# Draghoyns/FLAIR-1

Measured on AMD Instinct MI355X. Metric: 512x512x5 tiles/s (train fwd+bwd), higher is better.
Workload: dtype bf16; 1 GPU; U-Net/ResNet34 5-ch 512x512 13-class train step (fwd + fused CE/argmax/confmat + bwd + SGD), bs=32/GPU, random-init weights; global_batch=32, parallelism=dp1, grad_allreduce=none

## Files before the change

flair-1_amd/csrc/conv_hg.hip:

```cpp
#include <stdlib.h>

#include "common.h"
#include "conv_route.h"
#include "halo_stage.h"
#include "launch.h"
#include "mma.h"
#include "tile_store.h"
#include "tune.h"

namespace flair {
namespace {

__device__ __forceinline__ int sw_off(int row, int chunk) { return row * 128 + ((chunk ^ (row & 7)) << 4); }

template <typename T, int TW, int TH, int BN, int HB, int TMv = 4>
struct HgCfg {
  static constexpr int CH = Elem<T>::CH;
  static constexpr int CK = 8 * CH;
  static constexpr int TPIX = TW * TH;
  static constexpr int HW_ = TW + 2, HH = TH + 2, HPIX = HW_ * HH;
  static constexpr int WMN = TPIX / (16 * TMv), WNN = BN / 64;
  static constexpr int NWAVE = WMN * WNN;
  static constexpr int NT = 64 * NWAVE;
  static constexpr int HALO = HPIX * 128;
// ... 169 lines not shown
#pragma unroll
  for (int q = 0; q < TN; ++q) {
    const int col = wn * 64 + q * 16 + lr;
    const bool cin_ok = (n0 + col) < a.Cout;
    const float osc = (a.oscale && cin_ok) ? a.oscale[n0 + col] : 1.f;
    const float bias = ((a.bias && cin_ok) ? a.bias[n0 + col] : 0.f) + ((a.oshift && cin_ok) ? a.oshift[n0 + col] : 0.f);
#pragma unroll
    for (int i = 0; i < TM; ++i) {
#pragma unroll
      for (int rr = 0; rr < 4; ++rr) {
        const int g = wm * TM + i;
        const int row = (g / MTX) * TW + (g % MTX) * 16 + lq * 4 + rr;
        T v = Elem<T>::from_f(fmaf(acc[i][q][rr], osc, bias));
        const float vf = Elem<T>::to_f(v);
        s1[q] += vf;
        s2[q] += vf * vf;
        *reinterpret_cast<T*>(ct + row * Cfg::CLD + col * (int)sizeof(T)) = v;
      }
    }
  }
  if (a.stats) {
#pragma unroll
    for (int q = 0; q < TN; ++q) {
      s1[q] += __shfl_xor(s1[q], 16); s1[q] += __shfl_xor(s1[q], 32);
      s2[q] += __shfl_xor(s2[q], 16); s2[q] += __shfl_xor(s2[q], 32);
      if (lq == 0) {
        st[(wm * BN + wn * 64 + q * 16 + lr) * 2 + 0] = s1[q];
        st[(wm * BN + wn * 64 + q * 16 + lr) * 2 + 1] = s2[q];
      }
    }
  }
  __syncthreads();
  if (a.stats) tile_stats_write<Cfg::WMN, BN>(st, a.stats, a.Cout, n0, ntiles, tile, t);
  store_tile<T, TW, TPIX, BN, NT, Cfg::CLD, BNR>(a, ct, n, y0, x0, n0, t, tile, ntiles);
}

void* g_debug_buffer = nullptr;
typedef const __attribute__((address_space(1))) void* gptr_t;
typedef __attribute__((address_space(3))) void* lptr_t;

template <typename T, int TW, int TH, int BN, int HB, int NS>
struct HgdCfg {
  static constexpr int CH = Elem<T>::CH;
  static constexpr int CK = 8 * CH;
  static constexpr int TPIX = TW * TH;
  static constexpr int HW_ = TW + 2, HH = TH + 2, HPIX = HW_ * HH;
  static constexpr int WMN = TPIX / 64, WNN = BN >= 64 ? BN / 64 : 1;
  static constexpr int TN = BN / 16 / WNN;
  static constexpr int NWAVE = WMN * WNN;
  static constexpr int NT = 64 * NWAVE;
  static constexpr int HALO = HPIX * 128;
  static constexpr int BTILE = BN * 128;
  static constexpr int CLD = BN * (int)sizeof(T) + 16;
  static constexpr int CT = TPIX * CLD;
  static constexpr int STAGES = HB * HALO + NS * BTILE;
  static constexpr int MAIN = STAGES > CT ? STAGES : CT;
  static constexpr int STATS = WMN * BN * 2 * 4;
  static constexpr int SMEM = MAIN + STATS;
  static constexpr int HITEMS = (HPIX * 8 + NT - 1) / NT;
  static constexpr int DPW = BTILE / (1024 * NWAVE);
  static constexpr int D = NS - 1;
  static_assert(BTILE % (1024 * NWAVE) == 0, "every wave streams whole 1 KiB pieces");
  static_assert(D >= 1 && D <= 3, "ring depth");
};

__device__ __forceinline__ void wait_vm_lgkm0(int n) {
#define FLAIR_VM_CASE(k) case k: asm volatile("s_waitcnt vmcnt(" #k ") lgkmcnt(0)" ::: "memory"); break;
  switch (n) {
    FLAIR_VM_CASE(1) FLAIR_VM_CASE(2) FLAIR_VM_CASE(3) FLAIR_VM_CASE(4) FLAIR_VM_CASE(5) FLAIR_VM_CASE(6) FLAIR_VM_CASE(7)
    FLAIR_VM_CASE(8) FLAIR_VM_CASE(9) FLAIR_VM_CASE(10) FLAIR_VM_CASE(11) FLAIR_VM_CASE(12) FLAIR_VM_CASE(13)
    FLAIR_VM_CASE(14) FLAIR_VM_CASE(15) FLAIR_VM_CASE(16) FLAIR_VM_CASE(17) FLAIR_VM_CASE(18) FLAIR_VM_CASE(19)
    FLAIR_VM_CASE(20) FLAIR_VM_CASE(21) FLAIR_VM_CASE(22) FLAIR_VM_CASE(23) FLAIR_VM_CASE(24) FLAIR_VM_CASE(25)
    FLAIR_VM_CASE(26) FLAIR_VM_CASE(27) FLAIR_VM_CASE(28) FLAIR_VM_CASE(29) FLAIR_VM_CASE(30) FLAIR_VM_CASE(31)
    FLAIR_VM_CASE(32) FLAIR_VM_CASE(33) FLAIR_VM_CASE(34) FLAIR_VM_CASE(35) FLAIR_VM_CASE(36) FLAIR_VM_CASE(37)
    FLAIR_VM_CASE(38) FLAIR_VM_CASE(39) FLAIR_VM_CASE(40) FLAIR_VM_CASE(41) FLAIR_VM_CASE(42) FLAIR_VM_CASE(43)
    FLAIR_VM_CASE(44) FLAIR_VM_CASE(45) FLAIR_VM_CASE(46) FLAIR_VM_CASE(47) FLAIR_VM_CASE(48)
    default: asm volatile("s_waitcnt vmcnt(0) lgkmcnt(0)" ::: "memory"); break;
  }
#undef FLAIR_VM_CASE
}

enum { XF_NONE = 0, XF_LAZY = 1 };

template <typename T, int TW, int TH, int BN, int HB, int NS, bool BNR, int XF>
__global__ __launch_bounds__(TW * TH * (BN >= 64 ? BN : 64) / 64, 2) void conv3x3_hgd_kernel(const ConvArgs a) {
  constexpr bool LAZY = XF == XF_LAZY;
  using Cfg = HgdCfg<T, TW, TH, BN, HB, NS>;
  constexpr int CH = Cfg::CH, CK = Cfg::CK, HW_ = Cfg::HW_, HPIX = Cfg::HPIX, NT = Cfg::NT, TPIX = Cfg::TPIX;
  constexpr int TM = 4, TN = Cfg::TN, MTX = TW / 16, DPW = Cfg::DPW, D = Cfg::D, HITEMS = Cfg::HITEMS;
  extern __shared__ __attribute__((aligned(16))) unsigned char smem[];
  unsigned char* halo0 = smem;
  unsigned char* bt0 = smem + HB * Cfg::HALO;
  const int t = threadIdx.x, lane = t & 63;
  const int wave = __builtin_amdgcn_readfirstlane(t >> 6);
  const int lr = lane & 15, lq = lane >> 4;
  const int wm = wave % Cfg::WMN, wn = wave / Cfg::WMN;
  const int H = a.Hout, W = a.Wout;
  const int tiles_x = W / TW, tiles_y = H / TH;
  const int NB = a.Cout / BN;
  const int nwork = gridDim.x;
  int w = blockIdx.x;
  if (a.xcd_remap) {
    const int q = nwork >> 3, r = nwork & 7, xcd = w & 7;
    w = (xcd < r ? xcd * (q + 1) : r * (q + 1) + (xcd - r) * q) + (w >> 3);
  }
  const int tile = w / NB;
  const int ntiles = nwork / NB;
  int n, y0, x0;
  tile_decode<TW, TH>(tile, tiles_x, tiles_y, n, y0, x0);
  const int n0 = (w - tile * NB) * BN;
  const int Cin = a.C0 + a.C1;
  const T* __restrict__ src0 = (const T*)a.src0;
  const T* __restrict__ src1 = (const T*)a.src1;
  const unsigned char* __restrict__ wp = (const unsigned char*)a.w;
  const int Hs0 = a.up0 ? (H >> 1) : H, Ws0 = a.up0 ? (W >> 1) : W;
  const int nchunks = Cin / CK;

  u32x4 hreg[HITEMS];
  unsigned hbits = 0;
  float lsc[CH], lsh[CH];
  bool hlazy = false;
  auto halo_load = [&](int chunk) {
    const int cbase = chunk * CK;
    const bool use0 = cbase < a.C0;
    const T* __restrict__ base = use0 ? src0 : src1;
    const int Hs = use0 ? Hs0 : H, Ws = use0 ? Ws0 : W, Cs = use0 ? a.C0 : a.C1;
    const int sh = (use0 && a.up0) ? 1 : 0;
    const int coff = use0 ? cbase : cbase - a.C0;
    unsigned hb2 = 0;
#pragma unroll
    for (int k = 0; k < HITEMS; ++k) {
      const int it = t + NT * k;
      const int hp = it >> 3, ch = it & 7;
      const int hy = hp / HW_, hx = hp - hy * HW_;
      const int iy = y0 - 1 + hy, ix = x0 - 1 + hx;
      const bool ok = (it < HPIX * 8) && ((unsigned)iy < (unsigned)H) && ((unsigned)ix < (unsigned)W);
      const unsigned off = ok ? (unsigned)(((n * Hs + (iy >> sh)) * Ws + (ix >> sh)) * Cs + coff + ch * CH) : 0u;
      hreg[k] = *reinterpret_cast<const u32x4*>(base + off);
      hb2 |= (ok ? 1u : 0u) << k;
    }
    hbits = hb2;
    if constexpr (LAZY) {
      hlazy = use0 && a.in_scale != nullptr;
      const int c0 = hlazy ? coff + (t & 7) * CH : 0;
      const float* __restrict__ ps = hlazy ? a.in_scale : (const float*)a.w;
      const float* __restrict__ ph = hlazy ? a.in_shift : (const float*)a.w;
#pragma unroll
      for (int e = 0; e < CH; e += 4) {
        const float4 v1 = *reinterpret_cast<const float4*>(ps + c0 + e), v2 = *reinterpret_cast<const float4*>(ph + c0 + e);
        lsc[e] = v1.x; lsc[e + 1] = v1.y; lsc[e + 2] = v1.z; lsc[e + 3] = v1.w;
        lsh[e] = v2.x; lsh[e + 1] = v2.y; lsh[e + 2] = v2.z; lsh[e + 3] = v2.w;
      }
    }
  };
  constexpr int HLOADS = HITEMS + (LAZY ? 2 * (CH / 4) : 0);
  static_assert((D - 1) * DPW + HLOADS <= 48, "wait_vm_lgkm0 covers the largest count its two call sites (prologue, end of a "
                                              "tap step) request: the D - 1 younger weight tiles and the loads of one halo chunk");
  auto halo_store = [&](int buf) {
    unsigned char* hb = halo0 + buf * Cfg::HALO;
#pragma unroll
    for (int k = 0; k < HITEMS; ++k) {
      const int it = t + NT * k;
      if (it < HPIX * 8) {
        const int hp = it >> 3, hx = hp % HW_;
        u32x4 v = hreg[k];
        if constexpr (LAZY) {
          if (hlazy) v = chunk_bn_relu<T, u32x4>(v, lsc, lsh);
        }
        *reinterpret_cast<u32x4*>(hb + hp * 128 + (((it & 7) ^ (hx & 7)) << 4)) = v & (0u - ((hbits >> k) & 1u));
        if constexpr (LAZY) __builtin_amdgcn_sched_barrier(0);
      }
    }
  };
  const unsigned bvo = (unsigned)(((n0 + wave * (DPW * 8) + (lane >> 3)) * a.Kpad + (((lane & 7) ^ (lane >> 3)) * CH)) * (int)sizeof(T));
  const unsigned brow = (unsigned)(8 * a.Kpad * (int)sizeof(T));
  auto b_dma = [&](int chunk, int tap, int slot) {
    const unsigned char* gb = wp + (size_t)(unsigned)((tap * Cin + chunk * CK) * (int)sizeof(T));
    unsigned char* lb = bt0 + slot * Cfg::BTILE + wave * (DPW * 1024);
#pragma unroll
    for (int j = 0; j < DPW; ++j)
      __builtin_amdgcn_global_load_lds((gptr_t)(gb + (bvo + j * brow)), (lptr_t)(lb + j * 1024), 16, 0, 0);
  };

  f32x4_t acc[TM][TN];
#pragma unroll
  for (int i = 0; i < TM; ++i)
#pragma unroll
    for (int j = 0; j < TN; ++j) acc[i][j] = f32x4_t{0.f, 0.f, 0.f, 0.f};

  unsigned abase[3], bfo[TN];
#pragma unroll
  for (int sx = 0; sx < 3; ++sx) abase[sx] = (unsigned)((lr + sx) * 128 + ((lq ^ ((lr + sx) & 7)) << 4));
#pragma unroll
  for (int j = 0; j < TN; ++j) bfo[j] = (unsigned)sw_off(wn * 64 + j * 16 + lr, lq);
  static_assert(TM % MTX == 0, "a wave's M tiles start at a tile-row boundary");
  const unsigned wbase = (unsigned)((wm * TM / MTX) * HW_ * 128);

  const int nsteps = 9 * nchunks;
  auto stamp = [&](int i) {
#ifdef FLAIR_HG_STAMPS
    if (a.dbg && t == 0) a.dbg[(size_t)blockIdx.x * 8 + i] = i == 5 || i == 6 ? __builtin_amdgcn_s_memrealtime() : __builtin_amdgcn_s_memtime();
#else
    (void)i;
#endif
  };
  stamp(0);
  stamp(5);
  u32x4 afA[TM], bfA[TN], afB[TM], bfB[TN];
  auto rd = [&](u32x4 (&af)[TM], u32x4 (&bf)[TN], const unsigned char* hbuf, int slot, int tap, int h) {
    const unsigned char* bb = bt0 + slot * Cfg::BTILE;
    const unsigned char* hbr = hbuf + (tap / 3) * (HW_ * 128);
#pragma unroll
    for (int j = 0; j < TN; ++j) bf[j] = *reinterpret_cast<const u32x4*>(bb + (bfo[j] ^ (h << 6)));
#pragma unroll
    for (int i = 0; i < TM; ++i)
      af[i] = *reinterpret_cast<const u32x4*>(hbr + wbase + ((i / MTX) * HW_ + (i % MTX) * 16) * 128 + (abase[tap % 3] ^ (h << 6)));
  };
  auto mm = [&](const u32x4 (&af)[TM], const u32x4 (&bf)[TN]) {
#pragma unroll
    for (int i = 0; i < TM; ++i)
#pragma unroll
      for (int j = 0; j < TN; ++j) Mma<T>::run(bf[j], af[i], acc[i][j]);
  };
  halo_load(0);
#pragma unroll
  for (int d = 0; d < D; ++d)
    if (d < nsteps) b_dma(d / 9, d % 9, d % NS);
  halo_store(0);
  const bool pre1 = nchunks > 1;
  if (pre1) halo_load(1);
  wait_vm_lgkm0((D - 1) * DPW + (pre1 ? HLOADS : 0));
  __builtin_amdgcn_s_barrier();
  __builtin_amdgcn_sched_barrier(0);
  stamp(1);
  constexpr bool PIPE = sizeof(T) == 2 && !(LAZY && BN == 64);
  if constexpr (PIPE) rd(afA, bfA, halo0, 0, 0, 0);

  int sb = 0;
  for (int chunk = 0; chunk < nchunks; ++chunk) {
    const unsigned char* hb = halo0 + (HB == 2 ? (chunk & 1) : 0) * Cfg::HALO;
    const unsigned char* hbn = halo0 + (HB == 2 ? ((chunk + 1) & 1) : 0) * Cfg::HALO;
    const bool last = chunk == nchunks - 1;
#pragma unroll
    for (int tap = 0; tap < 9; ++tap) {
      const int cur = (9 % NS == 0) ? (tap % NS) : ((sb + tap) % NS);
      const int nxt = (9 % NS == 0) ? ((tap + 1) % NS) : ((sb + tap + 1) % NS);
      {
        const int tp = tap + D;
        const int pc = tp >= 9 ? chunk + 1 : chunk, pt = tp >= 9 ? tp - 9 : tp;
        const int pslot = (9 % NS == 0) ? (tp % NS) : ((sb + tp) % NS);
        if (pc < nchunks) b_dma(pc, pt, pslot);
      }
      if constexpr (PIPE) {
        rd(afB, bfB, hb, cur, tap, 1);
        mm(afA, bfA);
      } else {
        rd(afA, bfA, hb, cur, tap, 0);
        mm(afA, bfA);
        rd(afA, bfA, hb, cur, tap, 1);
        mm(afA, bfA);
      }
      bool halo_younger = false;
      if (tap == 8) {
        if constexpr (HB == 2) {
          if (!last) {
            halo_store((chunk + 1) & 1);
            if (chunk + 2 < nchunks) { halo_load(chunk + 2); halo_younger = true; }
          }
        }
      } else if (tap <= D - 2) {
        halo_younger = chunk + 1 < nchunks;
      }
      const int left = last ? 8 - tap : 9;
      const int groups = left < 1 ? 0 : ((left < D ? left : D) - 1);
      wait_vm_lgkm0(left < 1 ? 0 : groups * DPW + (halo_younger ? HLOADS : 0));
      __builtin_amdgcn_s_barrier();
      __builtin_amdgcn_sched_barrier(0);
      if (tap < 8) {
        if constexpr (PIPE) {
          rd(afA, bfA, hb, nxt, tap + 1, 0);
          mm(afB, bfB);
        }
      } else if (!last) {
        if constexpr (HB == 1) {
          halo_store(0);
          if (chunk + 2 < nchunks) halo_load(chunk + 2);
          if constexpr (PIPE) mm(afB, bfB);
          asm volatile("s_waitcnt lgkmcnt(0)" ::: "memory");
          __builtin_amdgcn_s_barrier();
          __builtin_amdgcn_sched_barrier(0);
          if constexpr (PIPE) rd(afA, bfA, hbn, nxt, 0, 0);
        } else if constexpr (PIPE) {
          rd(afA, bfA, hbn, nxt, 0, 0);
          mm(afB, bfB);
        }
      } else if constexpr (PIPE) {
        mm(afB, bfB);
      }
    }
    if (9 % NS != 0) sb = (sb + 9) % NS;
  }
  stamp(2);

  unsigned char* ct = smem;
  float* st = reinterpret_cast<float*>(smem + Cfg::MAIN);
  const bool want_stats = a.stats != nullptr;
  const bool affine = a.oscale != nullptr || a.bias != nullptr || a.oshift != nullptr;
#pragma unroll
  for (int q = 0; q < TN; ++q) {
    const int colb = wn * 64 + q * 16 + lq * 4;
    float osc[4], bia[4];
#pragma unroll
    for (int rr = 0; rr < 4; ++rr) { osc[rr] = 1.f; bia[rr] = 0.f; }
    if (affine) {
#pragma unroll
      for (int rr = 0; rr < 4; ++rr) {
        const int c = n0 + colb + rr;
        const bool ok = c < a.Cout;
        if (a.oscale && ok) osc[rr] = a.oscale[c];
        bia[rr] = ((a.bias && ok) ? a.bias[c] : 0.f) + ((a.oshift && ok) ? a.oshift[c] : 0.f);
      }
    }
#pragma unroll
    for (int i = 0; i < TM; ++i) {
      const int g = wm * TM + i;
      const int row = (g / MTX) * TW + (g % MTX) * 16 + lr;
      float v[4];
#pragma unroll
      for (int rr = 0; rr < 4; ++rr) v[rr] = affine ? fmaf(acc[i][q][rr], osc[rr], bia[rr]) : acc[i][q][rr];
      if constexpr (sizeof(T) == 2) {
        uint2 pk;
        pk.x = (unsigned)f32_to_bf16(v[0]) | ((unsigned)f32_to_bf16(v[1]) << 16);
        pk.y = (unsigned)f32_to_bf16(v[2]) | ((unsigned)f32_to_bf16(v[3]) << 16);
        *reinterpret_cast<uint2*>(ct + row * Cfg::CLD + colb * 2) = pk;
      } else {
        *reinterpret_cast<float4*>(ct + row * Cfg::CLD + colb * 4) = make_float4(v[0], v[1], v[2], v[3]);
      }
    }
  }
  stamp(7);
  if (want_stats) {
    const unsigned char* cw = ct + (wm * 64) * Cfg::CLD + (wn * 64) * (int)sizeof(T);
#pragma unroll
    for (int q = 0; q < TN; ++q) {
      f32x4_t m1 = f32x4_t{0.f, 0.f, 0.f, 0.f}, m2 = f32x4_t{0.f, 0.f, 0.f, 0.f};
      if constexpr (sizeof(T) == 2) {
        typedef __attribute__((address_space(3))) s16x4_t* lds_p;
        const int p4 = lr & 3, q4 = lr >> 2;
#pragma unroll
        for (int ks = 0; ks < 2; ++ks) {
          const unsigned char* lo = cw + (ks * 32 + 8 * lq + q4) * Cfg::CLD + q * 32 + 8 * p4;
          const s16x4_t x0 = __builtin_amdgcn_ds_read_tr16_b64_v4i16((lds_p)(lo));
          const s16x4_t x1 = __builtin_amdgcn_ds_read_tr16_b64_v4i16((lds_p)(lo + 4 * Cfg::CLD));
          u32x4 xf;
          xf.x = (unsigned)(unsigned short)x0[0] | ((unsigned)(unsigned short)x0[1] << 16);
          xf.y = (unsigned)(unsigned short)x0[2] | ((unsigned)(unsigned short)x0[3] << 16);
          xf.z = (unsigned)(unsigned short)x1[0] | ((unsigned)(unsigned short)x1[1] << 16);
          xf.w = (unsigned)(unsigned short)x1[2] | ((unsigned)(unsigned short)x1[3] << 16);
          const u32x4 ones = u32x4{0x3F803F80u, 0x3F803F80u, 0x3F803F80u, 0x3F803F80u};
          Mma<T>::run(ones, xf, m1);
          Mma<T>::run(xf, xf, m2);
        }
      } else {
#pragma unroll
        for (int kk = 0; kk < 16; kk += 4) {
          u32x4 xf;
          xf.x = *reinterpret_cast<const unsigned*>(cw + ((kk + 0) * 4 + lq) * Cfg::CLD + (q * 16 + lr) * 4);
          xf.y = *reinterpret_cast<const unsigned*>(cw + ((kk + 1) * 4 + lq) * Cfg::CLD + (q * 16 + lr) * 4);
          xf.z = *reinterpret_cast<const unsigned*>(cw + ((kk + 2) * 4 + lq) * Cfg::CLD + (q * 16 + lr) * 4);
          xf.w = *reinterpret_cast<const unsigned*>(cw + ((kk + 3) * 4 + lq) * Cfg::CLD + (q * 16 + lr) * 4);
          const u32x4 ones = u32x4{0x3F800000u, 0x3F800000u, 0x3F800000u, 0x3F800000u};
          Mma<T>::run(ones, xf, m1);
          Mma<T>::run(xf, xf, m2);
        }
      }
      const int dr = lr & 3;
      const float d2 = dr == 0 ? m2[0] : dr == 1 ? m2[1] : dr == 2 ? m2[2] : m2[3];
      if (lq == 0) st[(wm * BN + wn * 64 + q * 16 + lr) * 2 + 0] = m1[0];
      if (lq == (lr >> 2)) st[(wm * BN + wn * 64 + q * 16 + lr) * 2 + 1] = d2;
    }
  }
  __syncthreads();
  if (a.stats) tile_stats_write<Cfg::WMN, BN>(st, a.stats, a.Cout, n0, ntiles, tile, t);
  stamp(3);
  store_tile<T, TW, TPIX, BN, NT, Cfg::CLD, BNR>(a, ct, n, y0, x0, n0, t, tile, ntiles);
  stamp(4);
  stamp(6);
}

static const char* hg_prof_name(size_t es, int BN) {
  static const char* names[2][3] = {{"conv3x3_hg_f32_n32", "conv3x3_hg_f32_n64", "conv3x3_hg_f32_n128"},
                                    {"conv3x3_hg_bf16_n32", "conv3x3_hg_bf16_n64", "conv3x3_hg_bf16_n128"}};
  return names[es == 2][BN == 128 ? 2 : BN == 64 ? 1 : 0];
}

template <typename T, int TW, int TH, int BN, int HB, int NS, bool BNR, int XF>
int launch_hgd_cfg_b(const ConvArgs& a, hipStream_t s) {
  using Cfg = HgdCfg<T, TW, TH, BN, HB, NS>;
  const long M = (long)a.N * a.Hout * a.Wout;
  dim3 grid((unsigned)(M / Cfg::TPIX) * (a.Cout / BN));
  ConvArgs b = a;
  b.xcd_remap = tune("FLAIR_XCD_REMAP", 1);
  b.dbg = (unsigned long long*)g_debug_buffer;
  return launch_kernel<conv3x3_hgd_kernel<T, TW, TH, BN, HB, NS, BNR, XF>>(hg_prof_name(sizeof(T), BN), conv_prof_cost(a, sizeof(T), true, false), grid,
                                                                           dim3(Cfg::NT), Cfg::SMEM, s, b);
}

template <typename T, int TW, int TH, int BN, int HB, int NS>
int launch_hgd_cfg(const ConvArgs& a, hipStream_t s) {
  if constexpr (BN == 32) {
    return (a.in_scale || a.bnr_partial) ? -6 : launch_hgd_cfg_b<T, TW, TH, BN, HB, NS, false, XF_NONE>(a, s);
  } else {
    if (a.in_scale) return a.bnr_partial ? -6 : launch_hgd_cfg_b<T, TW, TH, BN, HB, NS, false, XF_LAZY>(a, s);
    if constexpr (sizeof(T) == 2)
      return a.bnr_partial ? launch_hgd_cfg_b<T, TW, TH, BN, HB, NS, true, XF_NONE>(a, s)
                           : launch_hgd_cfg_b<T, TW, TH, BN, HB, NS, false, XF_NONE>(a, s);
    else
      return -6;
  }
}

int g_hg_variant = -1;

template <typename T, int TW, int TH, int BN, int HB, bool BNR, int TMv = 4>
int launch_hg_cfg_b(const ConvArgs& a, hipStream_t s) {
  using Cfg = HgCfg<T, TW, TH, BN, HB, TMv>;
  const long M = (long)a.N * a.Hout * a.Wout;
  dim3 grid((unsigned)(M / Cfg::TPIX) * (a.Cout / BN));
  ConvArgs b = a;
  b.xcd_remap = tune("FLAIR_XCD_REMAP", 1);
  return launch_kernel<conv3x3_hg_kernel<T, TW, TH, BN, HB, BNR, TMv>>(hg_prof_name(sizeof(T), BN), conv_prof_cost(a, sizeof(T), true, false), grid,
                                                                       dim3(Cfg::NT), Cfg::SMEM, s, b);
}

template <typename T, int TW, int TH, int BN, int HB, int TMv = 4>
int launch_hg_cfg(const ConvArgs& a, hipStream_t s) {
  return a.bnr_partial ? launch_hg_cfg_b<T, TW, TH, BN, HB, true, TMv>(a, s) : launch_hg_cfg_b<T, TW, TH, BN, HB, false, TMv>(a, s);
}

}

static int hg_dma_mode() { return tune("FLAIR_HG_DMA", 1); }

static int hg_tile_pixels(int dtype, const ConvArgs& a) {
  (void)dtype;
  if (g_hg_variant < 0) g_hg_variant = tune("FLAIR_HG_VARIANT", 1);
  const bool can128 = (a.Wout % 16 == 0) && (a.Hout % 8 == 0);
  const bool can256 = (a.Wout % 32 == 0 && a.Hout % 8 == 0) || (a.Wout % 16 == 0 && a.Hout % 16 == 0);
  if ((a.Cout % 128) != 0) return can256 ? 256 : (can128 ? 128 : 0);
  if (hg_dma_mode() == 0 && g_hg_variant == 0 && can256) return 256;
  if (can128) return 128;
  return can256 ? 256 : 0;
}

bool conv_hg_applicable(int dtype, const ConvArgs& a) {
  const int ck = dtype == DT_F32 ? 32 : 64;
  const int Cin = a.C0 + a.C1;
  if (a.R != 3 || a.S != 3 || a.out_mul != 1 || a.in_div != 1 || a.pad != 1) return false;
  if (a.Hout != a.Hin || a.Wout != a.Win || a.out_nchw || !a.out) return false;
  if (a.in_scale && (hg_dma_mode() == 0 || a.bnr_partial)) return false;
  if ((Cin % ck) || (a.C0 % ck)) return false;
  if (a.Cout == 32) return hg_dma_mode() != 0 && tune("FLAIR_HG_N32", 1) != 0 && !a.bnr_partial && !a.in_scale && a.pool_c0 == 0 &&
                           ((a.Wout % 32 == 0 && a.Hout % 8 == 0) || (a.Wout % 16 == 0 && a.Hout % 16 == 0));
  if (a.Cout < 64 || (a.Cout % 64)) return false;
  return hg_tile_pixels(dtype, a) != 0;
}

int conv_hg_grid_rows(int dtype, const ConvArgs& a) { return (int)((long)a.N * a.Hout * a.Wout / hg_tile_pixels(dtype, a)); }

template <typename T>
static int launch_hg_t(int tp, const ConvArgs& a, hipStream_t s) {
  const bool n128 = (a.Cout % 128) == 0;
  const int dma = hg_dma_mode();
  if (a.Cout == 32) {
    if (a.Wout % 32 == 0) return launch_hgd_cfg<T, 32, 8, 32, 1, 3>(a, s);
    return launch_hgd_cfg<T, 16, 16, 32, 1, 3>(a, s);
  }
  if (dma != 0 && (sizeof(T) == 2 || a.in_scale)) {
    if (tp == 128) return n128 ? launch_hgd_cfg<T, 16, 8, 128, 1, 3>(a, s) : launch_hgd_cfg<T, 16, 8, 64, 1, 3>(a, s);
    if (a.Wout % 32 == 0) return n128 ? launch_hgd_cfg<T, 32, 8, 128, 1, 3>(a, s) : launch_hgd_cfg<T, 32, 8, 64, 1, 3>(a, s);
    return n128 ? launch_hgd_cfg<T, 16, 16, 128, 1, 3>(a, s) : launch_hgd_cfg<T, 16, 16, 64, 1, 3>(a, s);
  }
  if (tp == 128) return n128 ? launch_hg_cfg<T, 16, 8, 128, 2>(a, s) : launch_hg_cfg<T, 16, 8, 64, 2>(a, s);
  if (a.Wout % 32 == 0) return n128 ? launch_hg_cfg<T, 32, 8, 128, 2>(a, s) : launch_hg_cfg<T, 32, 8, 64, 1>(a, s);
  return n128 ? launch_hg_cfg<T, 16, 16, 128, 2>(a, s) : launch_hg_cfg<T, 16, 16, 64, 1>(a, s);
}

int set_debug_buffer(void* p) {
#ifdef FLAIR_HG_STAMPS
  g_debug_buffer = p;
  return 0;
#else
  (void)p;
  return -7;
#endif
}

int launch_conv_hg(int dtype, const ConvArgs& a, hipStream_t s) {
  const int tp = hg_tile_pixels(dtype, a);
  return dtype == DT_F32 ? launch_hg_t<float>(tp, a, s) : launch_hg_t<bf16_t>(tp, a, s);
}

}
```

flair-1_amd/csrc/conv_igemm.hip:

```cpp
#include "common.h"
#include "conv_route.h"
#include "launch.h"
#include "mma.h"
#include "tile_store.h"
#include "tune.h"

namespace flair {

__device__ __forceinline__ int lds_off(int row, int chunk) { return row * 128 + ((chunk ^ (row & 7)) << 4); }

template <typename T, int BM, int BN, int WAVES_M, int WAVES_N>
struct ConvCfg {
  static constexpr int CH = Elem<T>::CH;
  static constexpr int BKE = 8 * CH;
  static constexpr int STAGE = (BM + BN) * 128;
  static constexpr int CLD = BN * (int)sizeof(T) + 16;
  static constexpr int CT = BM * CLD;
  static constexpr int MAIN = (2 * STAGE > CT) ? 2 * STAGE : CT;
  static constexpr int STATS = WAVES_M * BN * 2 * 4;
  static constexpr int SMEM = MAIN + STATS;
};

template <typename T, int BM, int BN, int WAVES_M, int WAVES_N>
__global__ __launch_bounds__(256, 2) void conv_igemm_kernel(const ConvArgs a) {
// ... 188 lines not shown
        uint4 v = *reinterpret_cast<const uint4*>(ct + row * Cfg::CLD + ch * 16);
        long mo = m;
        if (a.out_sub) {
          const int HWo = a.Hout * a.Wout;
          const int img = (int)(m / HWo), rem = (int)(m - (long)img * HWo);
          const int ho = rem / a.Wout, wo = rem - ho * a.Wout;
          mo = ((long)img * 2 * a.Hout + 2 * ho + c_oy) * (2 * a.Wout) + 2 * wo + c_ox;
        }
        T* dst = out + mo * a.out_ld + n;
        if (a.ores || a.orelu || a.ogelu) {
          float fa[CH];
          chunk_to_f<T>(v, fa);
          if (a.ogelu) {
#pragma unroll
            for (int e = 0; e < CH; ++e) fa[e] = 0.5f * fa[e] * (1.f + erff(fa[e] * 0.70710678118654752f));
          }
          if (a.ores) {
            float fb[CH];
            chunk_to_f<T>(*reinterpret_cast<const uint4*>((const T*)a.ores + mo * a.out_ld + n), fb);
#pragma unroll
            for (int e = 0; e < CH; ++e) fa[e] += fb[e];
          }
          if (a.orelu) {
#pragma unroll
            for (int e = 0; e < CH; ++e) fa[e] = fmaxf(fa[e], 0.f);
          }
          v = f_to_chunk<T>(fa);
        }
        if (a.accumulate) {
          uint4 o = *reinterpret_cast<const uint4*>(dst);
          float fa[CH], fb[CH];
          chunk_to_f<T>(v, fa);
          chunk_to_f<T>(o, fb);
#pragma unroll
          for (int e = 0; e < CH; ++e) fa[e] += fb[e];
          v = f_to_chunk<T>(fa);
        }
        *reinterpret_cast<uint4*>(dst) = v;
      }
    }
  }
  if (a.out_nchw) {
    const int HW = a.Hout * a.Wout;
    for (int idx = t; idx < BM * BN; idx += 256) {
      const int nl = idx / BM, ml = idx - nl * BM;
      const long m = m0 + ml;
      const int n = n0 + nl;
      if (m < M && n < a.Cout) {
        const long img = m / HW, pix = m - img * HW;
        a.out_nchw[(img * a.Cout + n) * HW + pix] =
            Elem<T>::to_f(*reinterpret_cast<const T*>(ct + ml * Cfg::CLD + nl * (int)sizeof(T)));
      }
    }
  }
}

template <typename T, int BM, int BN, int WAVES_M, int WAVES_N>
static int launch_cfg(const ConvArgs& a, hipStream_t s) {
  using Cfg = ConvCfg<T, BM, BN, WAVES_M, WAVES_N>;
  const long M = (long)a.N * a.Hout * a.Wout;
  dim3 grid(cdiv(M, BM), cdiv(a.Cout, BN), a.ncls ? a.ncls : 1);
  const double flops = 2.0 * (double)M * a.Cout * a.Kg / (a.in_div * a.in_div);
  const double bytes = ((double)a.N * a.Hin * a.Win / (a.in_div * a.in_div) / (a.up0 ? 4 : 1) * a.C0 +
                        (double)a.N * a.Hin * a.Win * a.C1 + (double)M * a.Cout * (a.accumulate ? 2 : 1)) * sizeof(T) +
                       (double)a.Cout * a.Kg * sizeof(T);
  static const char* names[2][4] = {{"conv_igemm_f32_128x128", "conv_igemm_f32_128x64", "conv_igemm_f32_256x32", "conv_igemm_f32_256x16"},
                                    {"conv_igemm_bf16_128x128", "conv_igemm_bf16_128x64", "conv_igemm_bf16_256x32", "conv_igemm_bf16_256x16"}};
  const int ci = BN == 128 ? 0 : BN == 64 ? 1 : BN == 32 ? 2 : 3;
  return launch_kernel<conv_igemm_kernel<T, BM, BN, WAVES_M, WAVES_N>>(names[sizeof(T) == 2][ci], ProfCost{flops, bytes}, grid, dim3(256), Cfg::SMEM, s, a);
}

static inline int pick_bn(int cout) { return cout >= 128 ? 128 : cout >= 64 ? 64 : cout >= 32 ? 32 : 16; }
static inline int pick_bm(int cout) { return cout >= 64 ? 128 : 256; }

ConvFamily conv_family(int dtype, const ConvArgs& a) {
  if (conv_stem_applicable(dtype, a)) return CONV_STEM;
  if (conv_hg_applicable(dtype, a)) return CONV_HG;
  if (conv_halo_applicable(a)) return CONV_HALO;
  return CONV_GATHER;
}

static bool tile_epilogue_ok(ConvFamily f, const ConvArgs& a) {
  if ((a.Hout & 1) || (a.Wout & 1)) return false;
  if (f == CONV_HG) return a.pool_c0 % ((a.Cout % 128) == 0 ? 128 : 64) == 0;
  if (f == CONV_HALO) return a.pool_c0 % (a.Cout <= 16 ? 16 : 32) == 0 && !a.out_nchw;
  return false;
}

bool conv_tile_epilogue_ok(int dtype, const ConvArgs& a) { return tile_epilogue_ok(conv_family(dtype, a), a); }

bool conv_mfma_bound(int dtype, const ConvArgs& a) {
  const int mode = tune("FLAIR_BNR", 2);
  if (mode == 0) return false;
  if (conv_family(dtype, a) != CONV_HG) return conv_halo_bnr_applicable(a);
  return mode == 2 || (a.Cout % 128) == 0;
}

bool conv_acc_src_ok(int dtype, const ConvArgs& a) { return a.acc_src && a.accumulate && a.pool_c0 == 0 && conv_family(dtype, a) == CONV_HG; }

int conv_grid_rows(int dtype, const ConvArgs& a) {
  switch (conv_family(dtype, a)) {
    case CONV_STEM: return conv_stem_grid_rows(a);
    case CONV_HG: return conv_hg_grid_rows(dtype, a);
    case CONV_HALO: return conv_halo_grid_rows(dtype, a);
    default: return cdiv((long)a.N * a.Hout * a.Wout, pick_bm(a.Cout));
  }
}

int conv_weight_rows_pad(int cout) { return (int)round_up(cout, pick_bn(cout)); }

template <typename T>
static int launch_t(const ConvArgs& a, hipStream_t s) {
  constexpr int CH = Elem<T>::CH;
  if ((a.C0 % CH) || (a.C1 % CH) || (a.Kpad % (8 * CH))) return -2;
  if (a.ncls && (a.ncls != 4 || !a.out_sub)) return -2;
  for (int c = 0; c < a.ncls; ++c)
    if (!a.cls_w[c] || (a.cls_kpad[c] % (8 * CH))) return -2;
  if (a.out && (a.Cout % CH)) return -3;
  if (a.up0 && ((a.Hin | a.Win) & 1)) return -4;
  if (a.in_div != 1 && a.in_div != 2) return -5;
  const long M = (long)a.N * a.Hout * a.Wout;
  const int bn = pick_bn(a.Cout);
  const bool small = !a.stats && !a.ncls && bn >= 64 && a.Kpad >= 8 * 8 * Elem<T>::CH && (long)cdiv(M, 128) * cdiv(a.Cout, bn) < 256 &&
                     tune("FLAIR_IGEMM_BM32", 2);
  if (small) {
    const int mode = tune("FLAIR_IGEMM_BM32", 2);
    if (mode >= 2 && (long)cdiv(M, 32) * cdiv(a.Cout, bn) < 512) return launch_cfg<T, 32, 32, 2, 2>(a, s);
    return bn == 128 ? launch_cfg<T, 32, 128, 2, 2>(a, s) : launch_cfg<T, 32, 64, 2, 2>(a, s);
  }
  switch (bn) {
    case 128: return launch_cfg<T, 128, 128, 2, 2>(a, s);
    case 64: return launch_cfg<T, 128, 64, 4, 1>(a, s);
    case 32: return launch_cfg<T, 256, 32, 4, 1>(a, s);
    default: return launch_cfg<T, 256, 16, 4, 1>(a, s);
  }
}

int launch_conv(int dtype, const ConvArgs& a, hipStream_t s) {
  const ConvFamily f = conv_family(dtype, a);
  if (a.preds_u8 && !conv_halo_preds_ok(dtype, a)) return -6;
  if (a.ce_lab8 && !conv_halo_ce_ok(dtype, a)) return -6;
  if (a.out_sub && (a.out_nchw || a.stats || a.pool_c0 > 0 || a.bnr_partial || f != CONV_GATHER)) return -6;
  if ((a.acc_src || a.bnr_mask) && f != CONV_HG) return -6;
  if (a.acc_src && !(a.accumulate && a.pool_c0 == 0)) return -6;
  if (a.bnr_mask && !a.bnr_partial) return -6;
  if (a.ogelu && (!a.out || a.out_nchw || a.in_scale || f != CONV_GATHER)) return -6;
  if (a.in_scale && ((f != CONV_HG && f != CONV_HALO) || (f == CONV_HG && (a.pool_c0 > 0 || a.bnr_partial)))) return -6;
  const bool tile_ok = tile_epilogue_ok(f, a);
  if (a.pool_c0 > 0 && !tile_ok) return -6;
  if (a.bnr_partial && !a.in_scale && !(tile_ok && (f == CONV_HG || conv_halo_bnr_applicable(a)))) return -6;
  switch (f) {
    case CONV_STEM: return launch_conv_stem(a, s);
    case CONV_HG: return launch_conv_hg(dtype, a, s);
    case CONV_HALO: {
      const int ch = dtype == DT_F32 ? 4 : 8;
      if (a.out && (a.Cout % ch) && a.out_ld < (int)round_up(a.Cout, ch)) return -3;
      return launch_conv_halo(dtype, a, s);
    }
    default: return dtype == DT_F32 ? launch_t<float>(a, s) : launch_t<bf16_t>(a, s);
  }
}

}
```

flair-1_amd/csrc/tile_store.h:

```cpp
#pragma once
#include "common.h"

namespace flair {

template <typename T, int TPIX, int BN, int NT>
struct TileItems {
  static constexpr int CH = Elem<T>::CH, CPR = BN / CH, ITEMS = (TPIX * CPR + NT - 1) / NT;
};

template <typename T, int TW, int TPIX, int BN, int NT>
__device__ __forceinline__ void tile_bnr_prefetch(const ConvArgs& a, int n, int y0, int x0, int n0, int t,
                                                  uint4 (&yv)[TileItems<T, TPIX, BN, NT>::ITEMS],
                                                  uint4 (&ov)[TileItems<T, TPIX, BN, NT>::ITEMS]) {
  using TI = TileItems<T, TPIX, BN, NT>;
  constexpr int CH = TI::CH, CPR = TI::CPR;
  const int H = a.Hout, W = a.Wout;
#pragma unroll
  for (int k = 0; k < TI::ITEMS; ++k) {
    const int idx = t + k * NT;
    const int row = idx / CPR, ch = idx - row * CPR;
    const int py = row / TW, px = row - py * TW;
    const int nn = n0 + ch * CH;
    const bool ok = idx < TPIX * CPR && nn < a.Cout;
    const long goff = ok ? ((long)(n * H + y0 + py) * W + x0 + px) * a.out_ld + nn : 0;
// ... 84 lines not shown
          float fb[CH];
          chunk_to_f<T>(*reinterpret_cast<const uint4*>(ct + row * CLD + ch * 16), fb);
#pragma unroll
          for (int e = 0; e < CH; ++e) fa[e] += fb[e];
        }
        T* dst = out + ((long)(n * Hh + (y0 >> 1) + py2) * Wh + (x0 >> 1) + px2) * a.out_ld + nn;
        if (a.accumulate) {
          float fb[CH];
          chunk_to_f<T>(*reinterpret_cast<const uint4*>(dst), fb);
#pragma unroll
          for (int e = 0; e < CH; ++e) fa[e] += fb[e];
        }
        uint4 v = f_to_chunk<T>(fa);
        if (bnr) v = bnr_item(v, *reinterpret_cast<const uint4*>((const T*)a.bnr_y + (dst - out)),
                              a.bnr_out ? *reinterpret_cast<const uint4*>((const T*)a.bnr_out + (dst - out)) : v);
        *reinterpret_cast<uint4*>(dst) = v;
      }
    }
    if (bnr) bnr_finish();
    return;
  }
  T* __restrict__ out = (T*)(a.pool_c0 > 0 ? a.out_skip : a.out);
  if (!out) return;
  const int ld = a.pool_c0 > 0 ? a.out_skip_ld : a.out_ld;
  const int cbase = a.pool_c0 > 0 ? a.pool_c0 : 0;
  const int acc = a.pool_c0 > 0 ? a.skip_accumulate : a.accumulate;
  constexpr int ITEMS = TileItems<T, TPIX, BN, NT>::ITEMS;
  uint4 yv[ITEMS], ov[ITEMS], av[ITEMS];
  if (bnr) tile_bnr_prefetch<T, TW, TPIX, BN, NT>(a, n, y0, x0, n0, t, yv, ov);
  const T* asrc = (a.acc_src && a.pool_c0 == 0) ? (const T*)a.acc_src : out;
  if (acc) {
#pragma unroll
    for (int k = 0; k < ITEMS; ++k) {
      const int idx = t + k * NT;
      const int row = idx / CPR, ch = idx - row * CPR;
      const int py = row / TW, px = row - py * TW;
      const int nn = n0 + ch * CH;
      const bool ok = idx < TPIX * CPR && nn < a.Cout;
      const long goff = ok ? ((long)(n * H + y0 + py) * W + x0 + px) * ld + (nn - cbase) : 0;
      av[k] = *reinterpret_cast<const uint4*>(asrc + goff);
    }
  }
#pragma unroll
  for (int k = 0; k < ITEMS; ++k) {
    const int idx = t + k * NT;
    if (idx >= TPIX * CPR) break;
    const int row = idx / CPR, ch = idx - row * CPR;
    const int py = row / TW, px = row - py * TW;
    const int nn = n0 + ch * CH;
    if (nn < a.Cout) {
      uint4 v = *reinterpret_cast<const uint4*>(ct + row * CLD + ch * 16);
      const long goff = ((long)(n * H + y0 + py) * W + x0 + px) * ld + (nn - cbase);
      T* dst = out + goff;
      if (a.ores || a.orelu) {
        float fa[CH];
        chunk_to_f<T>(v, fa);
        if (a.ores) {
          float fb[CH];
          chunk_to_f<T>(*reinterpret_cast<const uint4*>((const T*)a.ores + goff), fb);
#pragma unroll
          for (int e = 0; e < CH; ++e) fa[e] += fb[e];
        }
        if (a.orelu) {
#pragma unroll
          for (int e = 0; e < CH; ++e) fa[e] = fmaxf(fa[e], 0.f);
        }
        v = f_to_chunk<T>(fa);
      }
      if (acc) {
        float fa[CH], fb[CH];
        chunk_to_f<T>(v, fa);
        chunk_to_f<T>(av[k], fb);
#pragma unroll
        for (int e = 0; e < CH; ++e) fa[e] += fb[e];
        v = f_to_chunk<T>(fa);
      }
      if (bnr) v = bnr_item(v, yv[k], ov[k]);
      *reinterpret_cast<uint4*>(dst) = v;
    }
  }
  if (bnr) bnr_finish();
}

}
```

Measured before the change: 2835 tiles/s.

## Route stride-2 3x3 convs and their sub-pixel dgrad through the halo MFMA kernel

Adds stride-2 variants of the halo-DMA conv kernel. Forward stride-2 3x3 convs load the input as four polyphase sub-grids with a reordered tap table, so each halo chunk is reused across the taps of its phase. The backward data-gradient is split into four output-parity classes, each a small dense conv written by a new sub-pixel tile store. Both paths previously went through slower generic kernels; the new code adds more kernel instantiations and extra barriers at halo swaps.

```diff
diff --git a/flair-1_amd/csrc/conv_hg.hip b/flair-1_amd/csrc/conv_hg.hip
--- a/flair-1_amd/csrc/conv_hg.hip
+++ b/flair-1_amd/csrc/conv_hg.hip
@@ -275,9 +275,35 @@
 
 enum { XF_NONE = 0, XF_LAZY = 1 };
 
-template <typename T, int TW, int TH, int BN, int HB, int NS, bool BNR, int XF>
+enum { S2_NONE = 0, S2_FWD = 1, S2_DGRAD = 2 };
+constexpr int s2_period(int mode) { return mode == 0 ? 9 : mode == 1 ? 1 : mode == 4 ? 4 : 2; }
+constexpr int s2_groups(int mode) { return mode == 0 ? 4 : 1; }
+constexpr int s2_wtap(int mode, int k) {
+  constexpr int fwd[9] = {0, 2, 6, 8, 3, 5, 1, 7, 4};
+  return mode == 0 ? fwd[k] : k;
+}
+constexpr int s2_halo_tap(int mode, int k) {
+  if (mode == 0) return (s2_wtap(0, k) / 3 ? 3 : 0) + (s2_wtap(0, k) % 3 ? 1 : 0);
+  const int cs = ((mode - 1) & 1) ? 2 : 1;
+  return (1 + k / cs) * 3 + 1 + k % cs;
+}
+constexpr bool s2_group_end(int mode, int k) { return mode == 0 ? (k == 3 || k == 5 || k == 7 || k == 8) : k == s2_period(mode) - 1; }
+
+constexpr unsigned long long s2_pack(int mode, bool halo) {
+  unsigned long long v = 0;
+  for (int k = 0; k < s2_period(mode); ++k) v |= (unsigned long long)(halo ? s2_halo_tap(mode, k) : s2_wtap(mode, k)) << (4 * k);
+  return v;
+}
+constexpr unsigned s2_gmask(int mode) {
+  unsigned v = 0;
+  for (int k = 0; k < s2_period(mode); ++k) v |= (s2_group_end(mode, k) ? 1u : 0u) << k;
+  return v;
+}
+
+template <typename T, int TW, int TH, int BN, int HB, int NS, bool BNR, int XF, int S2 = S2_NONE>
 __global__ __launch_bounds__(TW * TH * (BN >= 64 ? BN : 64) / 64, 2) void conv3x3_hgd_kernel(const ConvArgs a) {
   constexpr bool LAZY = XF == XF_LAZY;
+  static_assert(S2 == S2_NONE || (HB == 1 && NS == 3 && !BNR && sizeof(T) == 2), "stride-2 flavours: single halo buffer, bf16");
   using Cfg = HgdCfg<T, TW, TH, BN, HB, NS>;
   constexpr int CH = Cfg::CH, CK = Cfg::CK, HW_ = Cfg::HW_, HPIX = Cfg::HPIX, NT = Cfg::NT, TPIX = Cfg::TPIX;
   constexpr int TM = 4, TN = Cfg::TN, MTX = TW / 16, DPW = Cfg::DPW, D = Cfg::D, HITEMS = Cfg::HITEMS;
@@ -305,7 +331,9 @@
   const int Cin = a.C0 + a.C1;
   const T* __restrict__ src0 = (const T*)a.src0;
   const T* __restrict__ src1 = (const T*)a.src1;
-  const unsigned char* __restrict__ wp = (const unsigned char*)a.w;
+  const int cls = S2 == S2_DGRAD ? 3 - (int)blockIdx.z : 0;
+  const unsigned char* __restrict__ wp = (const unsigned char*)(S2 == S2_DGRAD ? a.cls_w[cls] : a.w);
+  const int kpad = S2 == S2_DGRAD ? a.cls_kpad[cls] : a.Kpad;
   const int Hs0 = a.up0 ? (H >> 1) : H, Ws0 = a.up0 ? (W >> 1) : W;
   const int nchunks = Cin / CK;
 
@@ -313,9 +341,11 @@
   unsigned hbits = 0;
   float lsc[CH], lsh[CH];
   bool hlazy = false;
-  auto halo_load = [&](int chunk) {
-    const int cbase = chunk * CK;
-    const bool use0 = cbase < a.C0;
+  auto halo_load = [&](int chunk) __attribute__((always_inline)) {
+    const int pl = S2 == S2_FWD ? (chunk & 3) : 0;
+    const int pr = (pl & 1) ^ 1, pc = pl < 2 ? 1 : 0;
+    const int cbase = (S2 == S2_FWD ? (chunk >> 2) : chunk) * CK;
+    const bool use0 = S2 != S2_NONE || cbase < a.C0;
     const T* __restrict__ base = use0 ? src0 : src1;
     const int Hs = use0 ? Hs0 : H, Ws = use0 ? Ws0 : W, Cs = use0 ? a.C0 : a.C1;
     const int sh = (use0 && a.up0) ? 1 : 0;
@@ -327,8 +357,15 @@
       const int hp = it >> 3, ch = it & 7;
       const int hy = hp / HW_, hx = hp - hy * HW_;
       const int iy = y0 - 1 + hy, ix = x0 - 1 + hx;
-      const bool ok = (it < HPIX * 8) && ((unsigned)iy < (unsigned)H) && ((unsigned)ix < (unsigned)W);
-      const unsigned off = ok ? (unsigned)(((n * Hs + (iy >> sh)) * Ws + (ix >> sh)) * Cs + coff + ch * CH) : 0u;
+      bool ok = (it < HPIX * 8) && ((unsigned)iy < (unsigned)H) && ((unsigned)ix < (unsigned)W);
+      unsigned off;
+      if constexpr (S2 == S2_FWD) {
+        ok = ok && hy <= TH && hx <= TW && (hy >= 1 || pr) && (hx >= 1 || pc);
+        off = ok ? (unsigned)(((n * 2 * H + 2 * iy + pr) * (2 * W) + 2 * ix + pc) * Cs + coff + ch * CH) : 0u;
+      } else {
+        if constexpr (S2 == S2_DGRAD) ok = ok && hy >= 1 && hx >= 1;
+        off = ok ? (unsigned)(((n * Hs + (iy >> sh)) * Ws + (ix >> sh)) * Cs + coff + ch * CH) : 0u;
+      }
       hreg[k] = *reinterpret_cast<const u32x4*>(base + off);
       hb2 |= (ok ? 1u : 0u) << k;
     }
@@ -349,7 +386,7 @@
   constexpr int HLOADS = HITEMS + (LAZY ? 2 * (CH / 4) : 0);
   static_assert((D - 1) * DPW + HLOADS <= 48, "wait_vm_lgkm0 covers the largest count its two call sites (prologue, end of a "
                                               "tap step) request: the D - 1 younger weight tiles and the loads of one halo chunk");
-  auto halo_store = [&](int buf) {
+  auto halo_store = [&](int buf) __attribute__((always_inline)) {
     unsigned char* hb = halo0 + buf * Cfg::HALO;
 #pragma unroll
     for (int k = 0; k < HITEMS; ++k) {
@@ -365,9 +402,9 @@
       }
     }
   };
-  const unsigned bvo = (unsigned)(((n0 + wave * (DPW * 8) + (lane >> 3)) * a.Kpad + (((lane & 7) ^ (lane >> 3)) * CH)) * (int)sizeof(T));
-  const unsigned brow = (unsigned)(8 * a.Kpad * (int)sizeof(T));
-  auto b_dma = [&](int chunk, int tap, int slot) {
+  const unsigned bvo = (unsigned)(((n0 + wave * (DPW * 8) + (lane >> 3)) * kpad + (((lane & 7) ^ (lane >> 3)) * CH)) * (int)sizeof(T));
+  const unsigned brow = (unsigned)(8 * kpad * (int)sizeof(T));
+  auto b_dma = [&](int chunk, int tap, int slot) __attribute__((always_inline)) {
     const unsigned char* gb = wp + (size_t)(unsigned)((tap * Cin + chunk * CK) * (int)sizeof(T));
     unsigned char* lb = bt0 + slot * Cfg::BTILE + wave * (DPW * 1024);
 #pragma unroll
@@ -400,7 +437,7 @@
   stamp(0);
   stamp(5);
   u32x4 afA[TM], bfA[TN], afB[TM], bfB[TN];
-  auto rd = [&](u32x4 (&af)[TM], u32x4 (&bf)[TN], const unsigned char* hbuf, int slot, int tap, int h) {
+  auto rd = [&](u32x4 (&af)[TM], u32x4 (&bf)[TN], const unsigned char* hbuf, int slot, int tap, int h) __attribute__((always_inline)) {
     const unsigned char* bb = bt0 + slot * Cfg::BTILE;
     const unsigned char* hbr = hbuf + (tap / 3) * (HW_ * 128);
 #pragma unroll
@@ -409,12 +446,88 @@
     for (int i = 0; i < TM; ++i)
       af[i] = *reinterpret_cast<const u32x4*>(hbr + wbase + ((i / MTX) * HW_ + (i % MTX) * 16) * 128 + (abase[tap % 3] ^ (h << 6)));
   };
-  auto mm = [&](const u32x4 (&af)[TM], const u32x4 (&bf)[TN]) {
+  auto mm = [&](const u32x4 (&af)[TM], const u32x4 (&bf)[TN]) __attribute__((always_inline)) {
 #pragma unroll
     for (int i = 0; i < TM; ++i)
 #pragma unroll
       for (int j = 0; j < TN; ++j) Mma<T>::run(bf[j], af[i], acc[i][j]);
   };
+  constexpr bool PIPE = sizeof(T) == 2 && !(LAZY && BN == 64) && !(S2 == S2_FWD && BN == 64);
+  if constexpr (S2 != S2_NONE) {
+  static_assert(D == 2, "the look-ahead below is written for the ring of three");
+  unsigned long long wtab = s2_pack(0, false), htab = s2_pack(0, true);
+  unsigned gmask = s2_gmask(0);
+  int P = s2_period(0);
+  if constexpr (S2 == S2_DGRAD) {
+    P = cls == 0 ? s2_period(1) : cls == 3 ? s2_period(4) : s2_period(2);
+    wtab = s2_pack(4, false);
+    htab = cls == 0 ? s2_pack(1, true) : cls == 1 ? s2_pack(2, true) : cls == 2 ? s2_pack(3, true) : s2_pack(4, true);
+    gmask = 1u << (P - 1);
+  }
+  auto wtap_of = [&](int k) __attribute__((always_inline)) { return (int)((wtab >> (4 * k)) & 15); };
+  auto htap_of = [&](int k) __attribute__((always_inline)) { return (int)((htab >> (4 * k)) & 15); };
+  auto rdr = [&](u32x4 (&af)[TM], u32x4 (&bf)[TN], int slot, int htap, int h) __attribute__((always_inline)) {
+    const int hr = htap >= 6 ? 2 : htap >= 3 ? 1 : 0, hs = htap - 3 * hr;
+    const unsigned asel = (hs == 0 ? abase[0] : hs == 1 ? abase[1] : abase[2]) ^ (unsigned)(h << 6);
+    const unsigned char* bb = bt0 + slot * Cfg::BTILE;
+    const unsigned char* hbr = halo0 + hr * (HW_ * 128) + wbase;
+#pragma unroll
+    for (int j = 0; j < TN; ++j) bf[j] = *reinterpret_cast<const u32x4*>(bb + (bfo[j] ^ (h << 6)));
+#pragma unroll
+    for (int i = 0; i < TM; ++i) af[i] = *reinterpret_cast<const u32x4*>(hbr + ((i / MTX) * HW_ + (i % MTX) * 16) * 128 + asel);
+  };
+  const int nst = P * nchunks, nhalo = (S2 == S2_FWD ? s2_groups(0) : 1) * nchunks;
+  halo_load(0);
+  b_dma(0, wtap_of(0), 0);
+  if (nst > 1) b_dma(P == 1 ? 1 : 0, wtap_of(P == 1 ? 0 : 1), 1);
+  halo_store(0);
+  bool hyoung = nhalo > 1;
+  if (hyoung) halo_load(1);
+  wait_vm_lgkm0((nst > 1 ? DPW : 0) + (hyoung ? HLOADS : 0));
+  __builtin_amdgcn_s_barrier();
+  __builtin_amdgcn_sched_barrier(0);
+  if constexpr (PIPE) rdr(afA, bfA, 0, htap_of(0), 0);
+  int q = 0, k = 0, slot = 0, hidx = 0;
+#pragma unroll 1
+  for (int left = nst - 1; left >= 0; --left) {
+    int k1 = k + 1, q1 = q;
+    if (k1 == P) { k1 = 0; ++q1; }
+    int k2 = k1 + 1, q2 = q1;
+    if (k2 == P) { k2 = 0; ++q2; }
+    const int nxt = slot + 1 == NS ? 0 : slot + 1, pslot = nxt + 1 == NS ? 0 : nxt + 1;
+    if (q2 < nchunks) b_dma(q2, wtap_of(k2), pslot);
+    const int htap = htap_of(k);
+    if constexpr (PIPE) {
+      rdr(afB, bfB, slot, htap, 1);
+      mm(afA, bfA);
+    } else {
+      rdr(afA, bfA, slot, htap, 0);
+      mm(afA, bfA);
+      rdr(afA, bfA, slot, htap, 1);
+      mm(afA, bfA);
+    }
+    wait_vm_lgkm0(left < 1 ? 0 : (left >= D ? DPW : 0) + (hyoung ? HLOADS : 0));
+    hyoung = false;
+    __builtin_amdgcn_s_barrier();
+    __builtin_amdgcn_sched_barrier(0);
+    const bool sw = ((gmask >> k) & 1u) != 0 && left >= 1;
+    if (sw) {
+      halo_store(0);
+      ++hidx;
+      if (hidx + 1 < nhalo) { halo_load(hidx + 1); hyoung = true; }
+    } else if (left >= 1) {
+      if constexpr (PIPE) rdr(afA, bfA, nxt, htap_of(k1), 0);
+    }
+    if constexpr (PIPE) mm(afB, bfB);
+    if (sw) {
+      asm volatile("s_waitcnt lgkmcnt(0)" ::: "memory");
+      __builtin_amdgcn_s_barrier();
+      __builtin_amdgcn_sched_barrier(0);
+      if constexpr (PIPE) rdr(afA, bfA, nxt, htap_of(k1), 0);
+    }
+    k = k1; q = q1; slot = nxt;
+  }
+  } else {
   halo_load(0);
 #pragma unroll
   for (int d = 0; d < D; ++d)
@@ -426,7 +539,6 @@
   __builtin_amdgcn_s_barrier();
   __builtin_amdgcn_sched_barrier(0);
   stamp(1);
-  constexpr bool PIPE = sizeof(T) == 2 && !(LAZY && BN == 64);
   if constexpr (PIPE) rd(afA, bfA, halo0, 0, 0, 0);
 
   int sb = 0;
@@ -493,6 +605,7 @@
     }
     if (9 % NS != 0) sb = (sb + 9) % NS;
   }
+  }
   stamp(2);
 
   unsigned char* ct = smem;
@@ -576,7 +689,8 @@
   __syncthreads();
   if (a.stats) tile_stats_write<Cfg::WMN, BN>(st, a.stats, a.Cout, n0, ntiles, tile, t);
   stamp(3);
-  store_tile<T, TW, TPIX, BN, NT, Cfg::CLD, BNR>(a, ct, n, y0, x0, n0, t, tile, ntiles);
+  if constexpr (S2 == S2_DGRAD) store_tile_sub<T, TW, TPIX, BN, NT, Cfg::CLD>(a, ct, n, y0, x0, n0, t, cls >> 1, cls & 1);
+  else store_tile<T, TW, TPIX, BN, NT, Cfg::CLD, BNR>(a, ct, n, y0, x0, n0, t, tile, ntiles);
   stamp(4);
   stamp(6);
 }
@@ -613,6 +727,32 @@
   }
 }
 
+template <int TW, int TH, int BN>
+int launch_hgd_s2(const ConvArgs& a, hipStream_t s) {
+  using T = bf16_t;
+  using Cfg = HgdCfg<T, TW, TH, BN, 1, 3>;
+  const long M = (long)a.N * a.Hout * a.Wout;
+  const unsigned nwork = (unsigned)(M / Cfg::TPIX) * (a.Cout / BN);
+  ConvArgs b = a;
+  b.xcd_remap = tune("FLAIR_XCD_REMAP", 1);
+  b.dbg = (unsigned long long*)g_debug_buffer;
+  const double wbytes = (double)a.Cout * 9.0 * a.C0 * sizeof(T);
+  if (a.out_sub) {
+    for (int cls = 0; cls < 4; ++cls)
+      if (!a.cls_w[cls] || a.cls_kpad[cls] != ((cls >> 1) ? 2 : 1) * ((cls & 1) ? 2 : 1) * a.C0) return -2;
+    const ProfCost cost{2.0 * (double)M * a.Cout * 9.0 * a.C0,
+                        ((double)M * a.C0 + 4.0 * (double)M * a.Cout * (a.accumulate ? 2 : 1)) * sizeof(T) + wbytes};
+    return launch_kernel<conv3x3_hgd_kernel<T, TW, TH, BN, 1, 3, false, XF_NONE, S2_DGRAD>>("conv3x3_hg_bf16_s2_dgrad", cost, dim3(nwork, 1, 4),
+                                                                                          dim3(Cfg::NT), Cfg::SMEM, s, b);
+  }
+  const ProfCost cost{2.0 * (double)M * a.Cout * 9.0 * a.C0, (4.0 * (double)M * a.C0 + (double)M * a.Cout * (a.accumulate ? 2 : 1)) * sizeof(T) + wbytes};
+  if (a.in_scale)
+    return launch_kernel<conv3x3_hgd_kernel<T, TW, TH, BN, 1, 3, false, XF_LAZY, S2_FWD>>("conv3x3_hg_bf16_s2", cost, dim3(nwork), dim3(Cfg::NT),
+                                                                                        Cfg::SMEM, s, b);
+  return launch_kernel<conv3x3_hgd_kernel<T, TW, TH, BN, 1, 3, false, XF_NONE, S2_FWD>>("conv3x3_hg_bf16_s2", cost, dim3(nwork), dim3(Cfg::NT),
+                                                                                       Cfg::SMEM, s, b);
+}
+
 int g_hg_variant = -1;
 
 template <typename T, int TW, int TH, int BN, int HB, bool BNR, int TMv = 4>
@@ -635,8 +775,29 @@
 
 static int hg_dma_mode() { return tune("FLAIR_HG_DMA", 1); }
 
+static int hg_s2_form(int dtype, const ConvArgs& a) {
+  const bool fwd = a.R == 3 && a.S == 3 && a.out_mul == 2 && a.in_div == 1 && a.pad == 1 && !a.out_sub && !a.ncls &&
+                   a.Hin == 2 * a.Hout && a.Win == 2 * a.Wout;
+  const bool dgrad = a.out_sub && a.ncls == 4 && a.R == 2 && a.S == 2 && a.out_mul == 1 && a.in_div == 1 && a.pad == 0 &&
+                     a.Hin == a.Hout && a.Win == a.Wout;
+  if (!fwd && !dgrad) return S2_NONE;
+  const int mode = tune("FLAIR_HG_S2", 1);
+  if (dtype != DT_BF16 || hg_dma_mode() == 0 || mode == 0) return S2_NONE;
+  if (a.C1 || a.up0 || (a.C0 % 64) || a.Cout < 64 || (a.Cout % 64) || !a.out || a.out_ld < a.Cout || a.out_nchw) return S2_NONE;
+  if ((a.Wout % 16) || (a.Hout % 8)) return S2_NONE;
+  if (a.pool_c0 || a.bnr_partial || a.bnr_mask || a.acc_src || a.preds_u8 || a.ce_lab8 || a.ogelu) return S2_NONE;
+  if (dgrad && (a.in_scale || a.stats || a.bias || a.oscale || a.oshift || a.ores || a.orelu)) return S2_NONE;
+  if (mode == 1) {
+    if (fwd && a.C0 != 64) return S2_NONE;
+    const bool wide = (a.Cout % 128) == 0;
+    const long tiles = (long)a.N * a.Hout * a.Wout / ((!wide && (a.Wout % 32) == 0) ? 256 : 128);
+    if (tiles * (a.Cout / (wide ? 128 : 64)) * (dgrad ? 4 : 1) < 256) return S2_NONE;
+  }
+  return fwd ? S2_FWD : S2_DGRAD;
+}
+
 static int hg_tile_pixels(int dtype, const ConvArgs& a) {
-  (void)dtype;
+  if (hg_s2_form(dtype, a) != S2_NONE) return ((a.Cout % 128) != 0 && (a.Wout % 32) == 0) ? 256 : 128;
   if (g_hg_variant < 0) g_hg_variant = tune("FLAIR_HG_VARIANT", 1);
   const bool can128 = (a.Wout % 16 == 0) && (a.Hout % 8 == 0);
   const bool can256 = (a.Wout % 32 == 0 && a.Hout % 8 == 0) || (a.Wout % 16 == 0 && a.Hout % 16 == 0);
@@ -649,6 +810,7 @@
 bool conv_hg_applicable(int dtype, const ConvArgs& a) {
   const int ck = dtype == DT_F32 ? 32 : 64;
   const int Cin = a.C0 + a.C1;
+  if (hg_s2_form(dtype, a) != S2_NONE) return true;
   if (a.R != 3 || a.S != 3 || a.out_mul != 1 || a.in_div != 1 || a.pad != 1) return false;
   if (a.Hout != a.Hin || a.Wout != a.Win || a.out_nchw || !a.out) return false;
   if (a.in_scale && (hg_dma_mode() == 0 || a.bnr_partial)) return false;
@@ -691,6 +853,10 @@
 
 int launch_conv_hg(int dtype, const ConvArgs& a, hipStream_t s) {
   const int tp = hg_tile_pixels(dtype, a);
+  if (hg_s2_form(dtype, a) != S2_NONE) {
+    if ((a.Cout % 128) == 0) return launch_hgd_s2<16, 8, 128>(a, s);
+    return tp == 256 ? launch_hgd_s2<32, 8, 64>(a, s) : launch_hgd_s2<16, 8, 64>(a, s);
+  }
   return dtype == DT_F32 ? launch_hg_t<float>(tp, a, s) : launch_hg_t<bf16_t>(tp, a, s);
 }
 
diff --git a/flair-1_amd/csrc/conv_igemm.hip b/flair-1_amd/csrc/conv_igemm.hip
--- a/flair-1_amd/csrc/conv_igemm.hip
+++ b/flair-1_amd/csrc/conv_igemm.hip
@@ -294,6 +294,7 @@
 
 static bool tile_epilogue_ok(ConvFamily f, const ConvArgs& a) {
   if ((a.Hout & 1) || (a.Wout & 1)) return false;
+  if (a.out_sub || a.out_mul != 1) return false;
   if (f == CONV_HG) return a.pool_c0 % ((a.Cout % 128) == 0 ? 128 : 64) == 0;
   if (f == CONV_HALO) return a.pool_c0 % (a.Cout <= 16 ? 16 : 32) == 0 && !a.out_nchw;
   return false;
@@ -304,11 +305,14 @@
 bool conv_mfma_bound(int dtype, const ConvArgs& a) {
   const int mode = tune("FLAIR_BNR", 2);
   if (mode == 0) return false;
+  if (a.out_sub || a.out_mul != 1) return false;
   if (conv_family(dtype, a) != CONV_HG) return conv_halo_bnr_applicable(a);
   return mode == 2 || (a.Cout % 128) == 0;
 }
 
-bool conv_acc_src_ok(int dtype, const ConvArgs& a) { return a.acc_src && a.accumulate && a.pool_c0 == 0 && conv_family(dtype, a) == CONV_HG; }
+bool conv_acc_src_ok(int dtype, const ConvArgs& a) {
+  return a.acc_src && a.accumulate && a.pool_c0 == 0 && !a.out_sub && a.out_mul == 1 && conv_family(dtype, a) == CONV_HG;
+}
 
 int conv_grid_rows(int dtype, const ConvArgs& a) {
   switch (conv_family(dtype, a)) {
@@ -352,7 +356,7 @@
   const ConvFamily f = conv_family(dtype, a);
   if (a.preds_u8 && !conv_halo_preds_ok(dtype, a)) return -6;
   if (a.ce_lab8 && !conv_halo_ce_ok(dtype, a)) return -6;
-  if (a.out_sub && (a.out_nchw || a.stats || a.pool_c0 > 0 || a.bnr_partial || f != CONV_GATHER)) return -6;
+  if (a.out_sub && (a.out_nchw || a.stats || a.pool_c0 > 0 || a.bnr_partial || (f != CONV_GATHER && f != CONV_HG))) return -6;
   if ((a.acc_src || a.bnr_mask) && f != CONV_HG) return -6;
   if (a.acc_src && !(a.accumulate && a.pool_c0 == 0)) return -6;
   if (a.bnr_mask && !a.bnr_partial) return -6;
diff --git a/flair-1_amd/csrc/tile_store.h b/flair-1_amd/csrc/tile_store.h
--- a/flair-1_amd/csrc/tile_store.h
+++ b/flair-1_amd/csrc/tile_store.h
@@ -190,4 +190,45 @@
   if (bnr) bnr_finish();
 }
 
-}
+template <typename T, int TW, int TPIX, int BN, int NT, int CLD>
+__device__ __forceinline__ void store_tile_sub(const ConvArgs& a, const unsigned char* ct, int n, int y0, int x0, int n0, int t, int oy,
+                                               int ox) {
+  constexpr int CH = Elem<T>::CH, CPR = BN / CH, ITEMS = TileItems<T, TPIX, BN, NT>::ITEMS;
+  T* __restrict__ out = (T*)a.out;
+  if (!out) return;
+  const int H = a.Hout, W = a.Wout;
+  auto goff_of = [&](int idx, bool& ok) -> long {
+    const int row = idx / CPR, ch = idx - row * CPR;
+    const int py = row / TW, px = row - py * TW;
+    const int nn = n0 + ch * CH;
+    ok = idx < TPIX * CPR && nn < a.Cout;
+    return ok ? ((long)(n * 2 * H + 2 * (y0 + py) + oy) * (2 * W) + 2 * (x0 + px) + ox) * a.out_ld + nn : 0;
+  };
+  uint4 av[ITEMS];
+  if (a.accumulate) {
+#pragma unroll
+    for (int k = 0; k < ITEMS; ++k) {
+      bool ok;
+      av[k] = *reinterpret_cast<const uint4*>(out + goff_of(t + k * NT, ok));
+    }
+  }
+#pragma unroll
+  for (int k = 0; k < ITEMS; ++k) {
+    const int idx = t + k * NT;
+    bool ok;
+    const long goff = goff_of(idx, ok);
+    if (!ok) continue;
+    uint4 v = *reinterpret_cast<const uint4*>(ct + (idx / CPR) * CLD + (idx % CPR) * 16);
+    if (a.accumulate) {
+      float fa[CH], fb[CH];
+      chunk_to_f<T>(v, fa);
+      chunk_to_f<T>(av[k], fb);
+#pragma unroll
+      for (int e = 0; e < CH; ++e) fa[e] += fb[e];
+      v = f_to_chunk<T>(fa);
+    }
+    *reinterpret_cast<uint4*>(out + goff) = v;
+  }
+}
+
+}
```

Measured after the change: 2843 tiles/s, median of 6. About the same (+0.3%).
